# unanan/UNet_Nested4Tiny_Objects_Keypoints

Measured on AMD Instinct MI355X. Metric: images/sec (train step) UNet++ L=4 256x256, higher is better.
Workload: dtype f32

## Files before the change

### include/unetpp_hip.h

```cpp
#ifndef UNETPP_HIP_H
#define UNETPP_HIP_H

#include <stdint.h>

#ifdef __cplusplus
extern "C" {
#endif

#define UNETPP_ABI_VERSION 12
#define UNETPP_MAX_VIEWS 8

#define UNETPP_OK 0
#define UNETPP_EINVAL (-1)
#define UNETPP_ELAUNCH (-2)

typedef struct unetpp_view {
  float* ptr;
  int32_t C, c_off, c_len;
  int32_t Hs, Ws;
  int32_t sy, sx, oy, ox;
  const float* scale;
  const float* shift;
  const float* gate;
  int32_t relu;
// ... 292 lines not shown
                      const int32_t* chunk_segment, int64_t n_chunks, int64_t count, double decay, float* count_dev,
                      const double* hyper_dev, int32_t* done, void* stream);

#define UNETPP_WARP_PARAMS 16
#define UNETPP_WARP_MAX_C 8
#define UNETPP_STORE_U8 0
#define UNETPP_STORE_F32 1

int unetpp_warp_batch(const void* store, int32_t store_type, int64_t M, int32_t Hs, int32_t Ws, int32_t C,
                      const int64_t* index, int32_t N, const float* params, const float* mul, const float* add,
                      float fill, float* out, int32_t Ho, int32_t Wo, const float* labels, int32_t S,
                      float* labels_out, uint8_t* inside, void* stream);

typedef struct unetpp_augment {
  float p_flip_h, p_flip_v;
  int32_t rot90;
  float max_deg;
  float scale_lo, scale_hi;
  float max_tx, max_ty;
  float gain_lo, gain_hi;
  float max_bias;
  int32_t reserved;
} unetpp_augment;

int unetpp_augment_draw(float* params, int32_t N, uint64_t seed, int32_t Hs, int32_t Ws, int32_t Ho, int32_t Wo,
                        const unetpp_augment* augment, void* stream);

#define UNETPP_SCENE_MAX_VARIANTS 8
#define UNETPP_SCENE_FLIP_X 1
#define UNETPP_SCENE_FLIP_Y 2
#define UNETPP_SCENE_TRANSPOSE 4

typedef struct unetpp_scene_rect {
  int32_t frame;
  int32_t oy, ox;
  int32_t y_lo, y_hi, x_lo, x_hi;
  int32_t reserved;
} unetpp_scene_rect;

int unetpp_scene_stitch(const float* tiles, int32_t n_tiles, int32_t K, int32_t C, int32_t Th, int32_t Tw,
                        const int32_t* variants, const unetpp_scene_rect* rects, const unetpp_scene_rect* rects_dev,
                        float* out, int32_t S, int32_t H, int32_t W, void* stream);


int64_t unetpp_peaks_workspace_bytes(int32_t M, int32_t H, int32_t W);
int unetpp_peaks_detect(const float* maps, int32_t M, int32_t H, int32_t W, float threshold, int32_t radius,
                        int32_t refine, int32_t cap, float* xy, float* score, int32_t* count, void* workspace,
                        void* stream);

int unetpp_detect_match(const float* xy, const int32_t* n_pred, const int32_t* order, int32_t S, int32_t C, int32_t cap,
                        const float* labels, const int32_t* label_class, int32_t L, float tolerance, int32_t* pred_label,
                        int32_t* label_pred, int32_t* stats, void* stream);

#ifdef __cplusplus
}
#endif
#endif
```

### unet_nested4tiny_objects_keypoints_amd/_lib.py

```python
from __future__ import annotations

import ctypes as C
import os
import subprocess

_PKG_DIR = os.path.dirname(os.path.abspath(__file__))
_REPO = os.path.dirname(_PKG_DIR)
LIB_PATH = os.environ.get("UNETPP_LIB", os.path.join(_PKG_DIR, "libunetpp_hip.so"))
CSRC = os.path.join(_PKG_DIR, "csrc")
INCLUDE = os.path.join(_REPO, "include")
SOURCES = ("gemm_pix.hip", "gemm_fast.hip", "gemm_pw.hip", "gemm_pw_bf16.hip", "gemm_wino.hip", "gemm_bf16.hip", "gemm_bf16_dma.hip", "wgrad_bf16.hip", "pointwise_bf16.hip", "keypoints.hip", "weight_image.hip", "wgrad.hip", "wgrad_fast.hip", "wgrad_dma.hip", "wgrad_pw.hip", "wgrad_wino.hip", "first_layer.hip", "pointwise.hip", "caller.hip", "optim.hip", "validate.hip", "average.hip", "loader.hip", "scene.hip",
           "detect.hip")
HEADERS = ("common.h", "gemm_units.h", "wgrad_reduce.h", "lds_asm.h", "bf16_common.h", "dropout.h", "bn_fused.h",
           "wino_experiments.h", "dma_experiments.h", "heads_mean.h")
MAX_VIEWS = 8
ABI_VERSION = 12
EXTRA_FLAGS = {"gemm_wino.hip": ("-fno-slp-vectorize",), "wgrad_wino.hip": ("-fno-slp-vectorize",)}
GEMM_DIRECT = 1
GEMM_BF16 = 2


class View(C.Structure):
    _fields_ = [
        ("ptr", C.c_void_p),
        ("C", C.c_int32), ("c_off", C.c_int32), ("c_len", C.c_int32),
        ("Hs", C.c_int32), ("Ws", C.c_int32),
        ("sy", C.c_int32), ("sx", C.c_int32), ("oy", C.c_int32), ("ox", C.c_int32),
        ("scale", C.c_void_p), ("shift", C.c_void_p), ("gate", C.c_void_p),
        ("relu", C.c_int32), ("accumulate", C.c_int32), ("gate_sum", C.c_int32), ("reserved", C.c_int32),
    ]


class BnFused(C.Structure):
    _fields_ = [
        ("gamma", C.c_void_p), ("beta", C.c_void_p), ("running_mean", C.c_void_p), ("running_var", C.c_void_p),
        ("mean", C.c_void_p), ("invstd", C.c_void_p), ("scale", C.c_void_p), ("shift", C.c_void_p),
        ("count", C.c_int64), ("eps", C.c_float), ("momentum", C.c_float),
    ]


class GemmDesc(C.Structure):
    _fields_ = [
        ("N", C.c_int32), ("H", C.c_int32), ("W", C.c_int32),
        ("taps", C.c_int32), ("n_in", C.c_int32), ("n_out", C.c_int32),
        ("flags", C.c_int32), ("reserved", C.c_int32),
        ("inp", View * MAX_VIEWS), ("out", View * MAX_VIEWS),
        ("weight", C.c_void_p), ("bias", C.c_void_p), ("stats_partial", C.c_void_p),
        ("weight_image", C.c_void_p),
        ("bn", BnFused),
    ]


class WeightSrc(C.Structure):
    _fields_ = [
        ("src", C.c_void_p),
        ("s_t", C.c_int64), ("s_k", C.c_int64), ("s_ko", C.c_int64), ("s_n", C.c_int64), ("s_no", C.c_int64),
        ("k_inner", C.c_int32), ("n_inner", C.c_int32), ("flip", C.c_int32), ("reserved", C.c_int32),
    ]


class PackJob(C.Structure):
    _fields_ = [
        ("src", WeightSrc),
        ("image", C.c_void_p),
        ("taps", C.c_int32), ("flags", C.c_int32), ("n_in", C.c_int32), ("n_out", C.c_int32),
# ... 125 lines not shown
    "unetpp_bn_bwd_reduce_pool": (C.c_int, [_P, _P, _P, _P, _P, _P, _P, _P, _I32, _I32, _I32, _I32, _P, _P]),
    "unetpp_bn_bwd_apply_pool": (C.c_int, [_P, _P, _P, _P, _P, _P, _P, _P, _P, _P, _P, _I32, _I32, _I32, _I32, _P, _P]),
    "unetpp_head_fwd": (C.c_int, [_P, _P, _P, _I32, _I32, _I32, _I32, _I32, _F, _U64, _P, _P, _P, _P]),
    "unetpp_head_bwd_blocks": (_I64, [_I64]),
    "unetpp_head_bwd": (C.c_int, [_P, _P, _P, _P, _I32, _I32, _I32, _I32, _I32, _F, _U64, _P, _P, _P, _I32, _I32, _P, _P]),
    "unetpp_sum_partials": (C.c_int, [_P, _I64, _I64, _P, _P]),
    "unetpp_focal_bce_blocks": (_I64, [_I64]),
    "unetpp_focal_bce": (C.c_int, [_P, _P, _I64, _I64, _F, _P, _P, _P, _P]),
    "unetpp_focal_bce_heads": (C.c_int, [C.POINTER(FocalHeads), _P, _I64, _I64, _F, _P, _P, _P]),
    "unetpp_heads_mean_fwd": (C.c_int, [C.POINTER(HeadsMean), _I32, _I32, _I32, _I32, _I32, _P, _P]),
    "unetpp_heads_mean_fwd_bf16": (C.c_int, [C.POINTER(HeadsMean), _I32, _I32, _I32, _I32, _I32, _P, _P]),
    "unetpp_bn_eval_coeffs_stats": (C.c_int, [_P, _P, _P, _P, _F, _I32, _P, _P, _P, _P, _P]),
    "unetpp_bn_frozen_bwd_blocks": (_I64, [_I64, _I32]),
    "unetpp_bn_frozen_bwd": (C.c_int, [_P, _P, _P, _P, _P, _P, _P, _P, _I32, _I32, _I32, _I32, _P, _P, _P]),
    "unetpp_bn_frozen_bwd_blocks_bf16": (_I64, [_I64, _I32]),
    "unetpp_bn_frozen_bwd_bf16": (C.c_int, [_P, _P, _P, _P, _P, _P, _P, _P, _I32, _I32, _I32, _I32, _P, _P, _P]),
    "unetpp_copy_jobs": (C.c_int, [_P, _I32, _I64, _P]),
    "unetpp_heatmap_workspace_bytes": (_I64, [_I32, _I32, _I32]),
    "unetpp_create_heatmap": (C.c_int, [_P, _I32, _I32, _I32, _I32, _F, _P, _P, _P]),
    "unetpp_bilinear2x_fwd": (C.c_int, [_P, _I32, _I32, _I32, _I32, _P, _P]),
    "unetpp_bilinear2x_bwd": (C.c_int, [_P, _I32, _I32, _I32, _I32, _P, _I32, _P]),
    "unetpp_nchw_to_nhwc": (C.c_int, [_P, _I32, _I32, _I32, _I32, _P, _P]),
    "unetpp_nhwc_to_nchw": (C.c_int, [_P, _I32, _I32, _I32, _I32, _P, _P]),
    "unetpp_affine_relu_pool_bf16": (C.c_int, [_P, _P, _P, _I32, _I32, _I32, _I32, _I32, _P, _P, _P, _P]),
    "unetpp_bn_bwd_blocks_bf16": (_I64, [_I64, _I32]),
    "unetpp_bn_bwd_reduce_bf16": (C.c_int, [_P, _P, _P, _P, _P, _P, _P, _P, _I32, _I32, _I32, _I32, _P, _P]),
    "unetpp_bn_bwd_apply_bf16": (C.c_int, [_P, _P, _P, _P, _P, _P, _P, _P, _P, _P, _P, _I32, _I32, _I32, _I32, _P, _P]),
    "unetpp_head_fwd_bf16": (C.c_int, [_P, _P, _P, _I32, _I32, _I32, _I32, _I32, _F, _U64, _P, _P, _P, _P]),
    "unetpp_first_layer_dgrad_bf16": (C.c_int, [_P, _P, _I32, _I32, _I32, _I32, _I32, _P, _P]),
    "unetpp_maxpool_bwd_bf16": (C.c_int, [_P, _P, _I32, _I32, _I32, _I32, _P, _P, _P]),
    "unetpp_bilinear2x_fwd_bf16": (C.c_int, [_P, _I32, _I32, _I32, _I32, _P, _P]),
    "unetpp_bilinear2x_bwd_bf16": (C.c_int, [_P, _I32, _I32, _I32, _I32, _P, _I32, _P, _P]),
    "unetpp_heatmap_pattern_workspace_bytes": (_I64, [_I32, _I32, _I32, _I32]),
    "unetpp_heatmap_pattern": (C.c_int, [_P, _I32, _I32, _P, _P, _I32, _I32, _I32, _F, _P, _P, _P]),
    "unetpp_keypoints_workspace_bytes": (_I64, [_I32, _I32, _I32, _I32]),
    "unetpp_keypoints_extract": (C.c_int, [_I32, _P, _I32, _I32, _I32, _P, _I32, _I32, _I32, _P, _P, _P, _P, _P]),
    "unetpp_head_bwd_bf16": (C.c_int, [_P, _P, _P, _P, _I32, _I32, _I32, _I32, _I32, _F, _U64, _P, _P, _P, _I32, _I32, _P, _P]),
    "unetpp_optim_chunk_elems": (_I64, []),
    "unetpp_optim_step": (C.c_int, [_I32, _I32, _P, _I32, _P, _I64, _P, _P, _P, _P]),
    "unetpp_optim_upload": (C.c_int, [_P, _P, _I64, _P]),
    "unetpp_match_points": (C.c_int, [_P, _P, _I32, _I32, _I32, _I32, _P, _I32, _P, _P, _P, _P, _P, _P, _P]),
    "unetpp_avg_update": (C.c_int, [_I32, _I32, _P, _I32, _P, _I64, _I64, C.c_double, _P, _P, _P, _P]),
    "unetpp_grad_norm": (C.c_int, [_P, _I32, _P, _I64, _P, _P]),
    "unetpp_optim_step_clip": (C.c_int, [_I32, _I32, _P, _I32, _P, _I64, _P, _P, _P, _P, _P, _P]),
    "unetpp_grad_scale": (C.c_int, [_P, _I32, _P, _I64, _P, _F, _P, _P]),
    "unetpp_warp_batch": (C.c_int, [_P, _I32, _I64, _I32, _I32, _I32, _P, _I32, _P, _P, _P, _F, _P, _I32, _I32, _P, _I32,
                                    _P, _P, _P]),
    "unetpp_augment_draw": (C.c_int, [_P, _I32, _U64, _I32, _I32, _I32, _I32, C.POINTER(AugmentDesc), _P]),
    "unetpp_scene_stitch": (C.c_int, [_P, _I32, _I32, _I32, _I32, _I32, C.POINTER(C.c_int32), C.POINTER(SceneRect), _P, _P,
                                      _I32, _I32, _I32, _P]),
    "unetpp_peaks_workspace_bytes": (_I64, [_I32, _I32, _I32]),
    "unetpp_peaks_detect": (C.c_int, [_P, _I32, _I32, _I32, _F, _I32, _I32, _I32, _P, _P, _P, _P, _P]),
    "unetpp_detect_match": (C.c_int, [_P, _P, _P, _I32, _I32, _I32, _P, _P, _I32, _F, _P, _P, _P, _P]),
}

_LIB = None


def source_hash() -> str:
    import hashlib
    h = hashlib.sha256()
    for path in [os.path.join(CSRC, s) for s in SOURCES + HEADERS] + [os.path.join(INCLUDE, "unetpp_hip.h")]:
        with open(path, "rb") as f:
            h.update(f.read())
    return h.hexdigest()[:16]


def build_library(force: bool = False, verbose: bool = False, out_path: str = None, obj_dir: str = None) -> str:
    srcs = [os.path.join(CSRC, s) for s in SOURCES]
    deps = srcs + [os.path.join(CSRC, h) for h in HEADERS] + [os.path.join(INCLUDE, "unetpp_hip.h")]
    lib_path = out_path or LIB_PATH
    if not force and os.path.exists(lib_path) and all(os.path.getmtime(lib_path) >= os.path.getmtime(d) for d in deps):
        return lib_path
    hipcc = os.environ.get("HIPCC", "/opt/rocm/bin/hipcc")
    common = [hipcc, "--offload-arch=gfx950", "-O3", "-std=c++17", "-fPIC", "-I", INCLUDE, "-I", CSRC]
    obj_dir = obj_dir or os.path.join(_REPO, "build", "obj")
    os.makedirs(obj_dir, exist_ok=True)
    jobs = []
    for src in SOURCES:
        obj = os.path.join(obj_dir, src.replace(".hip", ".o"))
        cmd = common + list(EXTRA_FLAGS.get(src, ())) + ["-c", os.path.join(CSRC, src), "-o", obj]
        if verbose:
            print(" ".join(cmd))
        jobs.append((obj, cmd, subprocess.Popen(cmd)))
    for obj, cmd, proc in jobs:
        if proc.wait() != 0:
            raise subprocess.CalledProcessError(proc.returncode, cmd)
    staged = os.path.join(obj_dir, os.path.basename(lib_path) + ".link")
    link = [hipcc, "--offload-arch=gfx950", "-shared", "-fPIC", "-o", staged] + [j[0] for j in jobs]
    if verbose:
        print(" ".join(link))
    subprocess.run(link, check=True)
    os.replace(staged, lib_path)
    if out_path is None:
        global _LIB
        _LIB = None
    return lib_path


def lib():
    global _LIB
    if _LIB is None:
        if not os.path.exists(LIB_PATH):
            raise RuntimeError(
                "unetpp HIP library not built: %s is missing. Run `python -c 'import __graft_entry__ as g; g.build()'` "
                "(there is no CPU fallback for this path)." % LIB_PATH)
# ... 37 lines not shown
```

### unet_nested4tiny_objects_keypoints_amd/engine.py

```python
from __future__ import annotations

import os

from typing import Dict, List, Optional, Tuple

import torch

from . import ops
from .ops import V


USE_PACK_PLAN = os.environ.get("UNETPP_NO_PACK_PLAN") is None
USE_GROUPED_DGRAD = os.environ.get("UNETPP_NO_GROUPED_DGRAD") is None
USE_PLAN_COPIES = os.environ.get("UNETPP_NO_PLAN_COPIES") is None
_A1_MATERIALIZE_BYTES = int(float(os.environ.get("UNETPP_BF16_A1_MAX_MB", "80")) * (1 << 20))
_A1_MATERIALIZE_BYTES_F32 = int(float(os.environ.get("UNETPP_F32_A1_MAX_MB", "80")) * (1 << 20))


def _empty(n, like):
    return torch.empty(n, dtype=torch.float32, device=like.device)


def _packed(w, t, k, n, dstr, sstr, flip=False):
    dst = _empty(t * k * n, w)
    ops.pack_weight(dst, w, t, k, n, dstr, sstr, flip=flip)
    return dst


def pack_conv_fwd(w):
    co, ci, kh, kw = w.shape
    t = kh * kw
    return ops.WSrc(w, t, ci, co, s_t=1, s_k=t, s_n=ci * t,
                    pack=lambda: _packed(w, t, ci, co, (ci * co, co, 1), (1, t, ci * t)))


def pack_conv_dgrad(w):
    co, ci, kh, kw = w.shape
    t = kh * kw
    return ops.WSrc(w, t, co, ci, s_t=1, s_k=ci * t, s_n=t, flip=True,
                    pack=lambda: _packed(w, t, co, ci, (co * ci, ci, 1), (1, ci * t, t), flip=True))


def pack_conv_dgrad_slice(w, c_off, c_len):
    co, ci, kh, kw = w.shape
    t = kh * kw
    flat = w.reshape(-1)[c_off * t:]
    return ops.WSrc(flat, t, co, c_len, s_t=1, s_k=ci * t, s_n=t, flip=True,
                    pack=lambda: _packed(w[:, c_off:c_off + c_len].contiguous(), t, co, c_len, (co * c_len, c_len, 1),
                                         (1, c_len * t, t), flip=True))


def pack_deconv_fwd(w):
    ci, co = w.shape[0], w.shape[1]
    return ops.WSrc(w, 1, ci, 4 * co, s_t=0, s_k=4 * co, s_n=4, s_no=1, n_inner=co,
                    pack=lambda: _packed(w, 4, ci, co, (co, 4 * co, 1), (1, 4 * co, 4)))


def pack_deconv_dgrad(w):
    ci, co = w.shape[0], w.shape[1]
    return ops.WSrc(w, 1, 4 * co, ci, s_t=0, s_k=4, s_ko=1, k_inner=co, s_n=4 * co,
                    pack=lambda: _packed(w, 4, co, ci, (co * ci, ci, 1), (1, 4, 4 * co)))


def tile_bias4(b):
    co = b.numel()
    plan = ops.current_plan()
    if plan is not None and USE_PLAN_COPIES and b.is_contiguous():
        dst, ready = plan.copy_for(("bias4", b.data_ptr()) + ops.phase_tag(plan.phase), plan.phase, (b.data_ptr(), co),
                                   lambda: (_empty(4 * co, b), [b], [(b, 0, 0, 4, co, 0, co)]))
# ... 355 lines not shown
                               _new_grad(bn.weight), _new_grad(bn.bias), pool=pool_grad)
    if not (bn.weight.requires_grad or bn.bias.requires_grad):
        return ops.bn_frozen_backward(d_act, y, scale, shift, None, None, d_act, pool=pool_grad, want_sums=False)
    return ops.bn_frozen_backward(d_act, y, scale, shift, mean, invstd, d_act, _new_grad(bn.weight), _new_grad(bn.bias),
                                  pool=pool_grad)


def _pair_bwd(blk, r: _PairRec, d_out, in_targets: Optional[List[V]], b, grads, pre_gated=False, pool_grad=None,
              flush=None, in_slice: Optional[Tuple[int, int]] = None):
    conv1, conv2 = getattr(blk.conv1, "0"), getattr(blk.conv2, "0")
    h, w = r.h, r.w
    if blk.is_batchnorm:
        bn1, bn2 = getattr(blk.conv1, "1"), getattr(blk.conv2, "1")
        grads[bn2.weight], grads[bn2.bias] = _bn_bwd(bn2, r.bn2, r.frozen2, d_out, r.y2, pool_grad)
        dy2 = V(d_out)
        mean, invstd, scale, shift = r.bn1
        if r.a1 is not None:
            _conv_wgrad(conv2, [V(r.a1)], [dy2], b, h, w, grads)
        else:
            _conv_wgrad(conv2, [V(r.y1, scale=scale, shift=shift, relu=True)], [dy2], b, h, w, grads)
        if flush is not None:
            flush()
        d_a1 = torch.empty_like(r.y1)
        ops.gemm_fwd(b, h, w, 9, [dy2], [V(d_a1)], pack_conv_dgrad(conv2.weight.detach()))
        grads[bn1.weight], grads[bn1.bias] = _bn_bwd(bn1, r.bn1, r.frozen1, d_a1, r.y1, None)
        dy1 = V(d_a1)
    else:
        dy2 = V(d_out) if pre_gated else V(d_out, gate=r.out)
        _conv_wgrad(conv2, [V(r.a1)], [dy2], b, h, w, grads)
        if flush is not None:
            flush()
        d_a1 = torch.empty_like(r.a1)
        ops.gemm_fwd(b, h, w, 9, [dy2], [V(d_a1, gate=r.a1)], pack_conv_dgrad(conv2.weight.detach()))
        dy1 = V(d_a1)
    _conv_wgrad(conv1, r.ins, [dy1], b, h, w, grads)
    if flush is not None:
        flush()
    if in_targets is not None:
        if dy1.t.dtype == torch.bfloat16 and in_targets[0].t.dtype == torch.float32:
            ops.first_layer_dgrad_bf16(dy1.t, conv1.weight.detach(), in_targets[0].t)
        elif in_slice is not None:
            ops.gemm_fwd(b, h, w, 9, [dy1], in_targets, pack_conv_dgrad_slice(conv1.weight.detach(), in_slice[0], in_slice[1]))
        else:
            ops.gemm_fwd(b, h, w, 9, [dy1], in_targets, pack_conv_dgrad(conv1.weight.detach()))
    return dy1


def _up_bwd(upmod, is_deconv, u: _UpRec, d_up, d_src, accumulate, gate, b, grads):
    hs, ws = u.h, u.w
    if is_deconv:
        ci, co = upmod.weight.shape[0], upmod.weight.shape[1]
        dw = _new_grad(upmod.weight)
        db = _new_grad(upmod.bias)
        ops.wgrad(b, hs, ws, 1, [V(u.src)], _phase_views(d_up), dw, (0, 4 * co, 4, 1), db, n_inner=co)
        grads[upmod.weight], grads[upmod.bias] = dw, db
        ops.gemm_fwd(b, hs, ws, 1, _phase_views(d_up), [V(d_src, accumulate=accumulate, gate=gate, gate_sum=True)],
                     pack_deconv_dgrad(upmod.weight.detach()))
    else:
        conv = getattr(upmod, "1")
        _conv_wgrad(conv, [V(u.interp)], [V(d_up)], b, 2 * hs, 2 * ws, grads)
        d_interp = torch.empty_like(u.interp)
        ops.gemm_fwd(b, 2 * hs, 2 * ws, 1, [V(d_up)], [V(d_interp)], pack_conv_dgrad(conv.weight.detach()))
        ops.bilinear2x_bwd(d_interp, d_src, accumulate, gate)


def _grouped_weights(model, refresh=False, plan=None):
    cache = getattr(model, "_grouped_dgrad_w", None)
    d = model.depth
    if cache is None or refresh:
        fresh = {}
        for i in range(d - 1):
            for jj in range(d - 1 - i):
                ws = [getattr(getattr(model, "up_concat%d%d" % (i, jc)).conv.conv1, "0").weight.detach()
                      for jc in range(jj + 1, d - i)]
                f = ws[0].shape[0]
                parts = [w[:, (1 + jj) * f:(2 + jj) * f] for w in ws]
                old = None if cache is None else cache.get((i, jj))
                if old is not None and not (old.device == parts[0].device and old.dtype == parts[0].dtype):
                    old = None
                if plan is not None and all(w.is_contiguous() and w.dtype == torch.float32 for w in ws):
                    key, sig = ("grouped", i, jj), tuple(w.data_ptr() for w in ws)
                    if old is not None and plan.knows_copy(key, "bwd", sig + (old.data_ptr(),)):
                        plan.copy_for(key, "bwd", sig + (old.data_ptr(),), None)
                        fresh[(i, jj)] = old
                        continue
                    buf = old if old is not None else torch.empty((len(ws) * f, f) + tuple(ws[0].shape[2:]),
                                                                   dtype=ws[0].dtype, device=ws[0].device)
                    t = ws[0].shape[2] * ws[0].shape[3]
                    items = [(w, (1 + jj) * f * t, q * f * f * t, f, f * t, w.shape[1] * t, f * t) for q, w in enumerate(ws)]
                    plan.copy_for(key, "bwd", sig + (buf.data_ptr(),), lambda: (buf, list(ws), items))
                    old = buf
                if old is not None:
                    torch.cat(parts, 0, out=old)
                    fresh[(i, jj)] = old
                else:
                    fresh[(i, jj)] = torch.cat(parts, 0).contiguous()
        cache = fresh
        model._grouped_dgrad_w = cache
    return cache


def backward_impl(model, s: _Saved, d_outs, want_input_grad: bool, grad_sink=None):
    if USE_GROUPED_DGRAD:
        _grouped_weights(model, refresh=True, plan=_plan_of(model) if (USE_PACK_PLAN and USE_PLAN_COPIES) else None)
    if not USE_PACK_PLAN:
        return _backward_impl(model, s, d_outs, want_input_grad, grad_sink)
# ... 140 lines not shown
```

### unet_nested4tiny_objects_keypoints_amd/ops.py

```python
from __future__ import annotations

import ctypes as C
import functools
import os
from dataclasses import dataclass
from typing import Optional, Sequence

import torch

from . import _lib
from ._lib import MAX_VIEWS, GemmDesc, PackJob, View, WeightSrc, WgradDesc, check


def _stream():
    return C.c_void_p(torch.cuda.current_stream().cuda_stream)


class LaunchTimer:

    def __init__(self):
        self.launches = []
        self.regions = []
        self.want_launches = True
        self.want_regions = True
# ... 404 lines not shown
                check(lib.unetpp_gemm_pack_weight_image(C.byref(d), _ptr(image), _stream()),
                      "unetpp_gemm_pack_weight_image")
            d.weight_image = image.data_ptr()
    if d.weight_image is None and from_src:
        packed = weight.packed()
        d.weight = packed.data_ptr()
    acc = sum(v.c_len for v in d.out[:d.n_out] if v.accumulate) + sum(v.c_len for v in d.out[:d.n_out] if v.gate)
    _timed_call(None, 2.0 * n * h * w * taps * k * nc,
                lambda: check(_lib.lib().unetpp_gemm_fwd(C.byref(d), _stream()), "unetpp_gemm_fwd"),
                (2.0 if d.flags & _lib.GEMM_BF16 else 4.0) * n * h * w * (k + nc + acc))


def first_layer_dgrad_bf16(dy: torch.Tensor, weight: torch.Tensor, dx: torch.Tensor) -> None:
    n, h, w, co = dy.shape
    ci = dx.shape[3]
    _need(dy, "dy", torch.bfloat16)
    _need(weight, "weight")
    _need(dx, "dx")
    if tuple(weight.shape) != (co, ci, 3, 3) or tuple(dx.shape[:3]) != (n, h, w):
        raise ValueError("shape mismatch")
    check(_lib.lib().unetpp_first_layer_dgrad_bf16(_ptr(dy), _ptr(weight), n, h, w, ci, co, _ptr(dx), _stream()),
          "unetpp_first_layer_dgrad_bf16")


def pack_weight(dst: torch.Tensor, src: torch.Tensor, t: int, k: int, n: int, dstr, sstr, flip: bool = False) -> None:
    _need(dst, "pack dst")
    _need(src, "pack src")
    check(_lib.lib().unetpp_pack_weight(_ptr(dst), _ptr(src), t, k, n, dstr[0], dstr[1], dstr[2],
                                        sstr[0], sstr[1], sstr[2], int(flip), _stream()), "unetpp_pack_weight")


def wgrad(n: int, h: int, w: int, taps: int, xs: Sequence[V], dys: Sequence[V], dw: Optional[torch.Tensor],
          dw_strides, db: Optional[torch.Tensor], n_inner: Optional[int] = None, target_blocks: int = 256,
          direct: bool = False) -> _lib.WgradSizes:
    lib = _lib.lib()
    d = WgradDesc()
    d.N, d.H, d.W, d.taps = n, h, w, taps
    d.n_x, d.n_dy = len(xs), len(dys)
    k = sum(v.fill(d.x[i]) for i, v in enumerate(xs))
    nc = sum(v.fill(d.dy[i]) for i, v in enumerate(dys))
    d.flags = (_lib.GEMM_DIRECT if (direct or not USE_WINOGRAD) else 0) | _storage_flag(dys, xs)
    plan = _lib.WgradSizes()
    check(lib.unetpp_wgrad_plan(C.byref(d), target_blocks, C.byref(plan)), "unetpp_wgrad_plan")
    slabs = torch.empty(plan.slab_floats, dtype=torch.float32, device=xs[0].t.device)
    d.n_split, d.slabs = plan.n_split, slabs.data_ptr()
    _timed_call(None, 2.0 * n * h * w * taps * k * nc,
                lambda: check(lib.unetpp_wgrad(C.byref(d), _stream()), "unetpp_wgrad"),
                (2.0 if d.flags & _lib.GEMM_BF16 else 4.0) * n * h * w * (k + nc))
    if n_inner is None:
        n_inner = nc
    check(lib.unetpp_wgrad_finish(_ptr(slabs), plan.n_split, plan.planes, k, nc, n_inner, _ptr(dw), dw_strides[0],
                                  dw_strides[1], dw_strides[2], dw_strides[3], _ptr(db), _stream()), "unetpp_wgrad_finish")
    return plan


def bn_finalize(partial, n_blocks, c, count, gamma, beta, eps, momentum, running_mean, running_var):
    dev = partial.device
    mean, invstd, scale, shift = (torch.empty(c, dtype=torch.float32, device=dev) for _ in range(4))
    check(_lib.lib().unetpp_bn_finalize(_ptr(partial), n_blocks, c, count, _ptr(gamma), _ptr(beta), eps, momentum,
                                        _ptr(running_mean), _ptr(running_var), _ptr(mean), _ptr(invstd), _ptr(scale),
                                        _ptr(shift), _stream()), "unetpp_bn_finalize")
    return mean, invstd, scale, shift


def bn_eval_coeffs(gamma, beta, running_mean, running_var, eps):
    c = gamma.numel()
    scale, shift = (torch.empty(c, dtype=torch.float32, device=gamma.device) for _ in range(2))
    check(_lib.lib().unetpp_bn_eval_coeffs(_ptr(gamma), _ptr(beta), _ptr(running_mean), _ptr(running_var), eps, c,
                                           _ptr(scale), _ptr(shift), _stream()), "unetpp_bn_eval_coeffs")
    return scale, shift


def bn_eval_coeffs_stats(gamma, beta, running_mean, running_var, eps):
    c = gamma.numel()
    mean, invstd, scale, shift = (torch.empty(c, dtype=torch.float32, device=gamma.device) for _ in range(4))
    check(_lib.lib().unetpp_bn_eval_coeffs_stats(_ptr(gamma), _ptr(beta), _ptr(running_mean), _ptr(running_var), eps, c,
                                                 _ptr(scale), _ptr(shift), _ptr(mean), _ptr(invstd), _stream()),
          "unetpp_bn_eval_coeffs_stats")
    return mean, invstd, scale, shift


def _is_bf16(t):
    return t.dtype == torch.bfloat16


def affine_relu_pool(y, scale, shift, relu, act, pooled, pool_idx):
    n, h, w, c = y.shape
    if _is_bf16(y):
        check(_lib.lib().unetpp_affine_relu_pool_bf16(_ptr(y), _ptr(scale), _ptr(shift), int(relu), n, h, w, c, _ptr(act),
                                                      _ptr(pooled), _ptr(pool_idx), _stream()),
              "unetpp_affine_relu_pool_bf16")
        return
    check(_lib.lib().unetpp_affine_relu_pool(_ptr(y), _ptr(scale), _ptr(shift), int(relu), n, h, w, c, _ptr(act),
                                             _ptr(pooled), _ptr(pool_idx), _stream()), "unetpp_affine_relu_pool")


def maxpool_bwd(d_pooled, pool_idx, d_act, gate=None):
    n, h, w, c = d_act.shape
    if _is_bf16(d_act):
        check(_lib.lib().unetpp_maxpool_bwd_bf16(_ptr(d_pooled), _ptr(pool_idx), n, h, w, c, _ptr(d_act), _ptr(gate), _stream()),
              "unetpp_maxpool_bwd_bf16")
        return
    if gate is not None:
        raise ValueError("the fused ReLU mask is a bf16-storage option")
    check(_lib.lib().unetpp_maxpool_bwd(_ptr(d_pooled), _ptr(pool_idx), n, h, w, c, _ptr(d_act), _stream()),
          "unetpp_maxpool_bwd")
# ... 548 lines not shown
```

Measured before the change: 1716.

## Fuse transposed-conv weight gradient and data gradient into one pointwise backward kernel

Adds a HIP kernel that computes the 2x2 stride-2 deconvolution's weight/bias gradient and its input gradient in a single pass. Each tile of the upsampled gradient and the source activation is read once and feeds both the wgrad MFMA accumulation and the dgrad MFMA with its gate/accumulate epilogue. Previously these were two launches that each read the same activations. In exchange it uses a large LDS footprint, an eight-wave in-block reduction and per-shape template variants. It applies only to f32 levels whose width is a multiple of 16 and whose weights fit in LDS.

```diff
diff --git a/include/unetpp_hip.h b/include/unetpp_hip.h
--- a/include/unetpp_hip.h
+++ b/include/unetpp_hip.h
@@ -368,6 +368,10 @@
                         const float* labels, const int32_t* label_class, int32_t L, float tolerance, int32_t* pred_label,
                         int32_t* label_pred, int32_t* stats, void* stream);
 
+
+int unetpp_pw_bwd_fused(const unetpp_wgrad_desc* d, const float* weight, const unetpp_view* d_src, int32_t launch,
+                        void* stream);
+
 #ifdef __cplusplus
 }
 #endif
diff --git a/unet_nested4tiny_objects_keypoints_amd/_lib.py b/unet_nested4tiny_objects_keypoints_amd/_lib.py
--- a/unet_nested4tiny_objects_keypoints_amd/_lib.py
+++ b/unet_nested4tiny_objects_keypoints_amd/_lib.py
@@ -10,7 +10,7 @@
 CSRC = os.path.join(_PKG_DIR, "csrc")
 INCLUDE = os.path.join(_REPO, "include")
 SOURCES = ("gemm_pix.hip", "gemm_fast.hip", "gemm_pw.hip", "gemm_pw_bf16.hip", "gemm_wino.hip", "gemm_bf16.hip", "gemm_bf16_dma.hip", "wgrad_bf16.hip", "pointwise_bf16.hip", "keypoints.hip", "weight_image.hip", "wgrad.hip", "wgrad_fast.hip", "wgrad_dma.hip", "wgrad_pw.hip", "wgrad_wino.hip", "first_layer.hip", "pointwise.hip", "caller.hip", "optim.hip", "validate.hip", "average.hip", "loader.hip", "scene.hip",
-           "detect.hip")
+           "detect.hip", "pw_bwd_fused.hip")
 HEADERS = ("common.h", "gemm_units.h", "wgrad_reduce.h", "lds_asm.h", "bf16_common.h", "dropout.h", "bn_fused.h",
            "wino_experiments.h", "dma_experiments.h", "heads_mean.h")
 MAX_VIEWS = 8
@@ -242,6 +242,7 @@
     "unetpp_peaks_workspace_bytes": (_I64, [_I32, _I32, _I32]),
     "unetpp_peaks_detect": (C.c_int, [_P, _I32, _I32, _I32, _F, _I32, _I32, _I32, _P, _P, _P, _P, _P]),
     "unetpp_detect_match": (C.c_int, [_P, _P, _P, _I32, _I32, _I32, _P, _P, _I32, _F, _P, _P, _P, _P]),
+    "unetpp_pw_bwd_fused": (C.c_int, [C.POINTER(WgradDesc), _P, C.POINTER(View), _I32, _P]),
 }
 
 _LIB = None
diff --git a/unet_nested4tiny_objects_keypoints_amd/csrc/pw_bwd_fused.hip b/unet_nested4tiny_objects_keypoints_amd/csrc/pw_bwd_fused.hip
--- /dev/null
+++ b/unet_nested4tiny_objects_keypoints_amd/csrc/pw_bwd_fused.hip
@@ -0,0 +1,362 @@
+#include "common.h"
+#include "lds_asm.h"
+
+namespace unetpp {
+namespace {
+
+constexpr int kFusedThreads = 512;
+constexpr size_t kFusedLdsBytes = 4 * 34 * 256 * sizeof(float);
+
+struct FusedArgs {
+  unetpp_wgrad_desc d;
+  unetpp_view out;
+  const float* weight;
+  int ci, co;
+  int kb_count, nb_count;
+  int nt_store;
+  long rows;
+};
+
+__device__ __forceinline__ long view_origin(const unetpp_view& v) {
+  return (static_cast<long>(v.oy) * v.Ws + v.ox) * v.C + v.c_off;
+}
+
+typedef unsigned u32x4v __attribute__((vector_size(16)));
+constexpr unsigned kBeyondRow = 0x80000000u;
+__device__ __forceinline__ __amdgpu_buffer_rsrc_t row_rsrc(const float* row, int row_bytes) {
+  return __builtin_amdgcn_make_buffer_rsrc(const_cast<float*>(row), 0, row_bytes, 0x00020000);
+}
+__device__ __forceinline__ f32x4 row_load4(__amdgpu_buffer_rsrc_t rs, unsigned lane_off, unsigned tile_off) {
+  return __builtin_bit_cast(f32x4, __builtin_amdgcn_raw_buffer_load_b128(rs, static_cast<int>(lane_off), static_cast<int>(tile_off), 0));
+}
+
+template <int NCB, bool FULL, bool GATE, bool ACC>
+__global__ __launch_bounds__(kFusedThreads, 2) void pw_bwd_fused_kernel(const FusedArgs a) {
+  constexpr int CO = 128 / NCB, NCH = 4 / NCB;
+  extern __shared__ __attribute__((aligned(16))) float fused_lds[];
+  const unetpp_wgrad_desc& d = a.d;
+  const int tid = threadIdx.x, lane = tid & 63, t16 = lane & 15, g = lane >> 4;
+  const int wave = __builtin_amdgcn_readfirstlane(tid >> 6);
+  constexpr int n_ps = 8;
+  const int ps = wave;
+  const int blocks = a.kb_count * a.nb_count, n_wg = gridDim.x;
+  int wg = blockIdx.x;
+  if ((n_wg & 7) == 0) wg = (blockIdx.x & 7) * (n_wg >> 3) + (blockIdx.x >> 3);
+  const int split = wg / blocks, sb = wg - split * blocks;
+  const int kb = sb / a.nb_count, nb = sb - kb * a.nb_count;
+  const int cb0 = sb * NCB;
+
+  for (int i = tid; i < 8 * NCH * NCB * 64; i += kFusedThreads) {
+    const int l = i & 63, blk = i >> 6;
+    const int cb = blk % NCB, qg = blk / NCB;
+    const int k = 16 * qg + 4 * (l >> 4), ph = k / CO, c = k - ph * CO;
+    const int n = 16 * (cb0 + cb) + (l & 15);
+    const float* wp = a.weight + (static_cast<long>(n) * CO + c) * 4 + ph;
+    *reinterpret_cast<f32x4*>(fused_lds + i * 4) = f32x4{wp[0], wp[4], wp[8], wp[12]};
+  }
+  __syncthreads();
+
+  const int W = d.W, H = d.H;
+  const unetpp_view& X0 = d.x[0];
+  const unetpp_view& Y0 = d.dy[0];
+  const unetpp_view& O = a.out;
+  const long x_row = static_cast<long>(X0.sy) * X0.Ws * X0.C, y_row = static_cast<long>(Y0.sy) * Y0.Ws * Y0.C;
+  const int x_px = X0.sx * X0.C, y_px = Y0.sx * Y0.C;
+  const int x_row_bytes = static_cast<int>(x_row) * 4, y_row_bytes = static_cast<int>(y_row) * 4;
+  const long x_org = view_origin(X0);
+  const int xa_c = static_cast<int>(x_org) + 64 * kb + 4 * t16;
+  int yb_c[2];
+#pragma unroll
+  for (int h = 0; h < 2; ++h) {
+    const int col = 128 * nb + 64 * h + 4 * t16, ph = col / CO;
+    yb_c[h] = static_cast<int>(view_origin(d.dy[ph])) + (col - ph * CO);
+  }
+  int yph[4];
+#pragma unroll
+  for (int p = 0; p < 4; ++p) yph[p] = static_cast<int>(view_origin(d.dy[p]));
+  const int o_px = O.sx * O.C;
+  const unsigned a_lane = static_cast<unsigned>(g * x_px + xa_c) * 4u;
+  const unsigned b_lane[2] = {static_cast<unsigned>(g * y_px + yb_c[0]) * 4u, static_cast<unsigned>(g * y_px + yb_c[1]) * 4u};
+  const bool o_gsum = O.gate_sum != 0;
+
+  const long parts = static_cast<long>(d.n_split) * n_ps, part = static_cast<long>(split) * n_ps + ps;
+  const long r0 = a.rows * part / parts, r1 = a.rows * (part + 1) / parts;
+
+  f32x4 acc[4][2][4];
+#pragma unroll
+  for (int m = 0; m < 4; ++m)
+#pragma unroll
+    for (int h = 0; h < 2; ++h)
+#pragma unroll
+      for (int q = 0; q < 4; ++q) acc[m][h][q] = f32x4{0.f, 0.f, 0.f, 0.f};
+  f32x4 dbs[2] = {f32x4{0.f, 0.f, 0.f, 0.f}, f32x4{0.f, 0.f, 0.f, 0.f}};
+
+  f32x4 X[8];
+  auto load_x = [&](auto chunk_c, long r, int x0) {
+    constexpr int chunk = decltype(chunk_c)::v;
+    const __amdgpu_buffer_rsrc_t yr = row_rsrc(Y0.ptr + r * y_row, y_row_bytes);
+    const unsigned lo = (FULL || x0 + t16 < W) ? static_cast<unsigned>(t16 * y_px + 4 * g) * 4u : kBeyondRow;
+#pragma unroll
+    for (int q = 0; q < 8; ++q) {
+      const int k0 = 128 * chunk + 16 * q, ph = k0 / CO, c = k0 - ph * CO;
+      X[q] = row_load4(yr, lo, static_cast<unsigned>(x0 * y_px + yph[ph] + c) * 4u);
+    }
+  };
+
+  const unsigned wa = lds_offset(fused_lds) + lane * 16;
+  long r = r0;
+  int x0 = 0;
+  if (r < r1) load_x(IC<0>{}, r, x0);
+  while (r < r1) {
+    const int n = static_cast<int>(r / H), y = static_cast<int>(r - static_cast<long>(n) * H);
+    const int x_this = x0;
+    const bool pv = FULL || x0 + t16 < W;
+    const __amdgpu_buffer_rsrc_t xr = row_rsrc(X0.ptr + r * x_row, x_row_bytes), yr = row_rsrc(Y0.ptr + r * y_row, y_row_bytes);
+    f32x4 A[4], B[4][2];
+#pragma unroll
+    for (int s = 0; s < 4; ++s) {
+      const unsigned lo = (FULL || x0 + 4 * s + g < W) ? a_lane : kBeyondRow;
+      A[s] = row_load4(xr, lo, static_cast<unsigned>((x0 + 4 * s) * x_px) * 4u);
+    }
+
+    const long o_tile = view_pixel_offset(O, n, y, x0) + 16 * cb0;
+    const __amdgpu_buffer_rsrc_t orr = row_rsrc(O.ptr + o_tile, 64 * o_px);
+    const __amdgpu_buffer_rsrc_t grr = row_rsrc(GATE ? O.gate + o_tile : O.ptr, 64 * o_px);
+    const unsigned oo = pv ? static_cast<unsigned>(t16 * o_px + 4 * g) * 4u : kBeyondRow;
+    constexpr bool kEarlyOld = NCB < 4;
+    f32x4 old[NCB];
+#pragma unroll
+    for (int cb = 0; cb < NCB; ++cb) {
+      if constexpr (ACC && kEarlyOld) old[cb] = row_load4(orr, oo, 64 * cb);
+    }
+
+    f32x4 dacc[NCB];
+#pragma unroll
+    for (int cb = 0; cb < NCB; ++cb) dacc[cb] = f32x4{0.f, 0.f, 0.f, 0.f};
+    static_for<NCH>([&](auto cc) {
+      constexpr int chunk = decltype(cc)::v;
+      if constexpr (chunk > 0) load_x(cc, r, x0);
+      const unsigned wb = wa + static_cast<unsigned>(chunk * (8 * NCB * 1024));
+      f32x4 wf[2];
+      asm volatile("ds_read_b128 %0, %1" : "=v"(wf[0]) : "v"(wb) : "memory");
+      static_for<8 * NCB>([&](auto ic) {
+        constexpr int i = decltype(ic)::v, q = i / NCB, cb = i % NCB;
+        if constexpr (i + 1 < 8 * NCB) {
+          asm volatile("ds_read_b128 %0, %1 offset:%2" : "=v"(wf[(i + 1) & 1]) : "v"(wb), "n"((i + 1) * 1024) : "memory");
+          asm volatile("s_waitcnt lgkmcnt(1)" : "+v"(wf[i & 1]));
+        } else {
+          asm volatile("s_waitcnt lgkmcnt(0)" : "+v"(wf[i & 1]));
+        }
+#pragma unroll
+        for (int e = 0; e < 4; ++e) dacc[cb] = __builtin_amdgcn_mfma_f32_16x16x4f32(wf[i & 1][e], X[q][e], dacc[cb], 0, 0, 0);
+      });
+    });
+
+    f32x4 gt[NCB];
+#pragma unroll
+    for (int cb = 0; cb < NCB; ++cb) {
+      if constexpr (GATE) gt[cb] = row_load4(grr, oo, 64 * cb);
+      if constexpr (ACC && !kEarlyOld) old[cb] = row_load4(orr, oo, 64 * cb);
+    }
+#pragma unroll
+    for (int cb = 0; cb < NCB; ++cb) {
+      f32x4 v = dacc[cb];
+      if constexpr (GATE) {
+#pragma unroll
+        for (int e = 0; e < 4; ++e) v[e] = (o_gsum || gt[cb][e] > 0.f) ? v[e] : 0.f;
+      }
+      if constexpr (ACC) {
+#pragma unroll
+        for (int e = 0; e < 4; ++e) v[e] += old[cb][e];
+      }
+      if constexpr (GATE) {
+#pragma unroll
+        for (int e = 0; e < 4; ++e) v[e] = (!o_gsum || gt[cb][e] > 0.f) ? v[e] : 0.f;
+      }
+      dacc[cb] = v;
+    }
+
+    auto load_b = [&]() {
+#pragma unroll
+      for (int s = 0; s < 4; ++s) {
+        const bool in_row = FULL || x_this + 4 * s + g < W;
+        const unsigned l0 = in_row ? b_lane[0] : kBeyondRow, l1 = in_row ? b_lane[1] : kBeyondRow;
+        B[s][0] = row_load4(yr, l0, static_cast<unsigned>((x_this + 4 * s) * y_px) * 4u);
+        B[s][1] = row_load4(yr, l1, static_cast<unsigned>((x_this + 4 * s) * y_px) * 4u);
+      }
+    };
+    if constexpr (kEarlyOld) load_b();
+#pragma unroll
+    for (int cb = 0; cb < NCB; ++cb) {
+      if (a.nt_store) __builtin_amdgcn_raw_buffer_store_b128(__builtin_bit_cast(u32x4v, dacc[cb]), orr, static_cast<int>(oo), 64 * cb, 2);
+      else __builtin_amdgcn_raw_buffer_store_b128(__builtin_bit_cast(u32x4v, dacc[cb]), orr, static_cast<int>(oo), 64 * cb, 0);
+    }
+    if constexpr (!kEarlyOld) load_b();
+
+    x0 += 16;
+    if (x0 >= W) {
+      x0 = 0;
+      ++r;
+    }
+    if (r < r1) load_x(IC<0>{}, r, x0);
+
+#pragma unroll
+    for (int s = 0; s < 4; ++s) {
+      if (FULL || x_this + 4 * s < W) {
+        const f32x4 av = A[s], b0 = B[s][0], b1 = B[s][1];
+#pragma unroll
+        for (int e = 0; e < 4; ++e) {
+          dbs[0][e] += b0[e];
+          dbs[1][e] += b1[e];
+        }
+#pragma unroll
+        for (int m = 0; m < 4; ++m)
+#pragma unroll
+          for (int q = 0; q < 4; ++q) {
+            acc[m][0][q] = __builtin_amdgcn_mfma_f32_16x16x4f32(av[m], b0[q], acc[m][0][q], 0, 0, 0);
+            acc[m][1][q] = __builtin_amdgcn_mfma_f32_16x16x4f32(av[m], b1[q], acc[m][1][q], 0, 0, 0);
+          }
+      }
+    }
+  }
+
+  float* red_lds = fused_lds;
+  for (int half = n_ps >> 1; half >= 1; half >>= 1) {
+    __syncthreads();
+    if (ps >= half && ps < 2 * half) {
+      float* rg = red_lds + (ps - half) * (34 * 256) + lane * 4;
+#pragma unroll
+      for (int m = 0; m < 4; ++m)
+#pragma unroll
+        for (int h = 0; h < 2; ++h)
+#pragma unroll
+          for (int q = 0; q < 4; ++q) *reinterpret_cast<f32x4*>(rg + ((m * 2 + h) * 4 + q) * 256) = acc[m][h][q];
+      *reinterpret_cast<f32x4*>(rg + 32 * 256) = dbs[0];
+      *reinterpret_cast<f32x4*>(rg + 33 * 256) = dbs[1];
+    }
+    __syncthreads();
+    if (ps < half) {
+      const float* rg = red_lds + ps * (34 * 256) + lane * 4;
+#pragma unroll
+      for (int m = 0; m < 4; ++m)
+#pragma unroll
+        for (int h = 0; h < 2; ++h)
+#pragma unroll
+          for (int q = 0; q < 4; ++q) acc[m][h][q] += *reinterpret_cast<const f32x4*>(rg + ((m * 2 + h) * 4 + q) * 256);
+      dbs[0] += *reinterpret_cast<const f32x4*>(rg + 32 * 256);
+      dbs[1] += *reinterpret_cast<const f32x4*>(rg + 33 * 256);
+    }
+  }
+  if (ps != 0) return;
+
+  const int Kw = a.ci, Nw = 4 * a.co;
+  float* slab = d.slabs + static_cast<long>(split) * (static_cast<long>(Kw) + 1) * Nw;
+#pragma unroll
+  for (int m = 0; m < 4; ++m)
+#pragma unroll
+    for (int h = 0; h < 2; ++h)
+#pragma unroll
+      for (int rr = 0; rr < 4; ++rr) {
+        const int k = 64 * kb + 4 * (4 * g + rr) + m, nn = 128 * nb + 64 * h + 4 * t16;
+        *reinterpret_cast<f32x4*>(slab + static_cast<long>(k) * Nw + nn) =
+            f32x4{acc[m][h][0][rr], acc[m][h][1][rr], acc[m][h][2][rr], acc[m][h][3][rr]};
+      }
+  if (kb == 0) {
+#pragma unroll
+    for (int h = 0; h < 2; ++h) {
+      f32x4 v = dbs[h];
+#pragma unroll
+      for (int e = 0; e < 4; ++e) {
+        v[e] += __shfl_xor(v[e], 16);
+        v[e] += __shfl_xor(v[e], 32);
+      }
+      if (g == 0) *reinterpret_cast<f32x4*>(slab + static_cast<long>(Kw) * Nw + 128 * nb + 64 * h + 4 * t16) = v;
+    }
+  }
+}
+
+bool fused_plain(const unetpp_view& v) {
+  return v.scale == nullptr && v.shift == nullptr && v.gate == nullptr && !v.relu && ((v.C | v.c_off | v.c_len) & 3) == 0 &&
+         (reinterpret_cast<uintptr_t>(v.ptr) & 15) == 0;
+}
+
+bool fused_shape(const unetpp_wgrad_desc* d, const float* weight, const unetpp_view* out, FusedArgs& a) {
+  if (d == nullptr || weight == nullptr || out == nullptr) return false;
+  if (d->N <= 0 || d->H <= 0 || d->W <= 0 || d->taps != 1 || (d->flags & UNETPP_GEMM_BF16) != 0) return false;
+  if (d->n_x != 1 || d->n_dy != 4 || d->slabs == nullptr || d->n_split < 1 || d->n_split > 4096) return false;
+  if ((reinterpret_cast<uintptr_t>(weight) & 3) != 0 || (reinterpret_cast<uintptr_t>(d->slabs) & 15) != 0) return false;
+  const unetpp_view& x = d->x[0];
+  if (!view_ok(x) || !view_covers(x, d->H, d->W) || !fused_plain(x) || x.Hs != x.sy * d->H) return false;
+  a.ci = x.c_len;
+  a.co = d->dy[0].c_len;
+  if ((a.ci & 63) != 0 || (a.co != 32 && a.co != 64 && a.co != 128)) return false;
+  for (int i = 0; i < 4; ++i) {
+    const unetpp_view& y = d->dy[i];
+    if (!view_ok(y) || !view_covers(y, d->H, d->W) || !fused_plain(y) || y.c_len != a.co || y.Hs != y.sy * d->H) return false;
+    if (y.ptr != d->dy[0].ptr || y.C != d->dy[0].C || y.Hs != d->dy[0].Hs || y.Ws != d->dy[0].Ws || y.sy != d->dy[0].sy ||
+        y.sx != d->dy[0].sx)
+      return false;
+  }
+  const unetpp_view& y0 = d->dy[0];
+  if (static_cast<long>(x.sy) * x.Ws * x.C * 4 >= 0x7fffffffL || static_cast<long>(y0.sy) * y0.Ws * y0.C * 4 >= 0x7fffffffL ||
+      static_cast<long>(out->sx) * out->C * 64 >= 0x7fffffffL)
+    return false;
+  if (!view_ok(*out) || !view_covers(*out, d->H, d->W) || out->c_len != a.ci || out->scale != nullptr || out->relu != 0) return false;
+  if (((out->C | out->c_off) & 3) != 0 || (reinterpret_cast<uintptr_t>(out->ptr) & 15) != 0 ||
+      (reinterpret_cast<uintptr_t>(out->gate) & 15) != 0)
+    return false;
+  a.kb_count = a.ci >> 6;
+  a.nb_count = a.co >> 5;
+  if (static_cast<long>(a.kb_count) * a.nb_count * d->n_split > 0x7fffffffL) return false;
+  a.rows = static_cast<long>(d->N) * d->H;
+  return true;
+}
+
+template <int NCB, bool FULL, bool GATE, bool ACC>
+int launch_fused(const FusedArgs& a, dim3 grid, hipStream_t st) {
+  static bool raised[64] = {};
+  int dev = 0;
+  if (hipGetDevice(&dev) != hipSuccess || dev < 0 || dev >= 64) return UNETPP_ELAUNCH;
+  if (!raised[dev]) {
+    if (hipFuncSetAttribute(reinterpret_cast<const void*>(&pw_bwd_fused_kernel<NCB, FULL, GATE, ACC>), hipFuncAttributeMaxDynamicSharedMemorySize,
+                            static_cast<int>(kFusedLdsBytes)) != hipSuccess)
+      return UNETPP_ELAUNCH;
+    raised[dev] = true;
+  }
+  hipLaunchKernelGGL((pw_bwd_fused_kernel<NCB, FULL, GATE, ACC>), grid, dim3(kFusedThreads), kFusedLdsBytes, st, a);
+  return launch_status();
+}
+
+}
+}
+
+using namespace unetpp;
+
+extern "C" int unetpp_pw_bwd_fused(const unetpp_wgrad_desc* d, const float* weight, const unetpp_view* d_src, int32_t launch,
+                                   void* stream) {
+  FusedArgs a;
+  if (!fused_shape(d, weight, d_src, a)) return UNETPP_EINVAL;
+  if (launch == 0) return UNETPP_OK;
+  a.d = *d;
+  a.out = *d_src;
+  a.weight = weight;
+  const long out_bytes = static_cast<long>(d->N) * d->H * d->W * a.ci * 4;
+  a.nt_store = static_cast<int>(opt_value(OPT_PW_NT, out_bytes >= (64L << 20) ? 1 : 0));
+  const dim3 grid(static_cast<unsigned>(d->n_split) * static_cast<unsigned>(a.kb_count * a.nb_count));
+  hipStream_t st = static_cast<hipStream_t>(stream);
+  note_kernel("pw_bwd_fused_kernel");
+  const bool full = (d->W & 15) == 0;
+  const bool gate = d_src->gate != nullptr, accum = d_src->accumulate != 0;
+#define UNETPP_FUSED_EPI(NCB, FULL) \
+  return gate ? (accum ? launch_fused<NCB, FULL, true, true>(a, grid, st) : launch_fused<NCB, FULL, true, false>(a, grid, st)) \
+              : (accum ? launch_fused<NCB, FULL, false, true>(a, grid, st) : launch_fused<NCB, FULL, false, false>(a, grid, st));
+#define UNETPP_FUSED_CASE(NCB) \
+  if (full) { UNETPP_FUSED_EPI(NCB, true) } else { UNETPP_FUSED_EPI(NCB, false) }
+  switch (a.co) {
+    case 32: UNETPP_FUSED_CASE(4)
+    case 64: UNETPP_FUSED_CASE(2)
+    default: UNETPP_FUSED_CASE(1)
+  }
+#undef UNETPP_FUSED_CASE
+#undef UNETPP_FUSED_EPI
+}
diff --git a/unet_nested4tiny_objects_keypoints_amd/engine.py b/unet_nested4tiny_objects_keypoints_amd/engine.py
--- a/unet_nested4tiny_objects_keypoints_amd/engine.py
+++ b/unet_nested4tiny_objects_keypoints_amd/engine.py
@@ -15,6 +15,11 @@
 USE_PLAN_COPIES = os.environ.get("UNETPP_NO_PLAN_COPIES") is None
 _A1_MATERIALIZE_BYTES = int(float(os.environ.get("UNETPP_BF16_A1_MAX_MB", "80")) * (1 << 20))
 _A1_MATERIALIZE_BYTES_F32 = int(float(os.environ.get("UNETPP_F32_A1_MAX_MB", "80")) * (1 << 20))
+USE_PW_FUSED_BWD = os.environ.get("UNETPP_PW_FUSED_BWD", "1") != "0"
+
+
+def _pw_fused_level(ci, co, ws):
+    return ws % 16 == 0 and (4 * co * ci + ci) * 4 <= 148 * 1024
 
 
 def _empty(n, like):
@@ -476,6 +481,11 @@
         ci, co = upmod.weight.shape[0], upmod.weight.shape[1]
         dw = _new_grad(upmod.weight)
         db = _new_grad(upmod.bias)
+        if (USE_PW_FUSED_BWD and _pw_fused_level(ci, co, ws) and d_up.dtype == torch.float32 and
+                ops.pw_bwd_fused(b, hs, ws, V(u.src), d_up, upmod.weight.detach(),
+                                 V(d_src, accumulate=accumulate, gate=gate, gate_sum=True), dw, db)):
+            grads[upmod.weight], grads[upmod.bias] = dw, db
+            return
         ops.wgrad(b, hs, ws, 1, [V(u.src)], _phase_views(d_up), dw, (0, 4 * co, 4, 1), db, n_inner=co)
         grads[upmod.weight], grads[upmod.bias] = dw, db
         ops.gemm_fwd(b, hs, ws, 1, _phase_views(d_up), [V(d_src, accumulate=accumulate, gate=gate, gate_sum=True)],
diff --git a/unet_nested4tiny_objects_keypoints_amd/ops.py b/unet_nested4tiny_objects_keypoints_amd/ops.py
--- a/unet_nested4tiny_objects_keypoints_amd/ops.py
+++ b/unet_nested4tiny_objects_keypoints_amd/ops.py
@@ -480,6 +480,47 @@
     check(lib.unetpp_wgrad_finish(_ptr(slabs), plan.n_split, plan.planes, k, nc, n_inner, _ptr(dw), dw_strides[0],
                                   dw_strides[1], dw_strides[2], dw_strides[3], _ptr(db), _stream()), "unetpp_wgrad_finish")
     return plan
+
+
+def pw_bwd_fused(n: int, h: int, w: int, src: V, d_up: torch.Tensor, weight: torch.Tensor, d_src: V,
+                 dw: torch.Tensor, db: torch.Tensor, target_blocks: int = 256) -> bool:
+    lib = _lib.lib()
+    ci, co = weight.shape[0], weight.shape[1]
+    _need(weight, "weight")
+    if tuple(weight.shape) != (ci, co, 2, 2) or d_up.dim() != 4 or tuple(d_up.shape) != (n, 2 * h, 2 * w, d_up.shape[3]):
+        raise ValueError("shape mismatch")
+    dys = [V(d_up, c_len=co, sy=2, sx=2, oy=a, ox=b) for a in (0, 1) for b in (0, 1)]
+    d = WgradDesc()
+    d.N, d.H, d.W, d.taps = n, h, w, 1
+    d.n_x, d.n_dy = 1, 4
+    k = src.fill(d.x[0])
+    nc = sum(v.fill(d.dy[i]) for i, v in enumerate(dys))
+    if src.t.dtype != torch.float32 or d_up.dtype != torch.float32 or d_src.t.dtype != torch.float32:
+        return False
+    d.flags = 0
+    out = View()
+    if d_src.fill(out) != ci or k != ci:
+        raise ValueError("src / d_src must have the weight's %d input channels" % ci)
+    plan = _lib.WgradSizes()
+    if lib.unetpp_wgrad_plan(C.byref(d), target_blocks, C.byref(plan)) == 0 and plan.kernel == b"wgrad_pw_kernel":
+        n_split = plan.n_split
+    else:
+        n_split = max(1, min(target_blocks // max(1, (ci // 64) * (co // 32)), n * h, 4096))
+    slabs = torch.empty(n_split * (ci + 1) * nc, dtype=torch.float32, device=d_up.device)
+    d.n_split, d.slabs = n_split, slabs.data_ptr()
+    if lib.unetpp_pw_bwd_fused(C.byref(d), _ptr(weight), C.byref(out), 0, None) != 0:
+        return False
+    _need(dw, "dw")
+    _need(db, "db")
+    if tuple(dw.shape) != (ci, co, 2, 2) or db.numel() != co:
+        raise ValueError("gradient shape mismatch")
+    acc = (ci if d_src.accumulate else 0) + (ci if d_src.gate is not None else 0)
+    _timed_call("pw_bwd_fused_kernel", 4.0 * n * h * w * ci * nc,
+                lambda: check(lib.unetpp_pw_bwd_fused(C.byref(d), _ptr(weight), C.byref(out), 1, _stream()),
+                              "unetpp_pw_bwd_fused"), 4.0 * n * h * w * (2 * ci + nc + acc))
+    check(lib.unetpp_wgrad_finish(_ptr(slabs), n_split, 1, ci, nc, co, _ptr(dw), 0, 4 * co, 4, 1, _ptr(db), _stream()),
+          "unetpp_wgrad_finish")
+    return True
 
 
 def bn_finalize(partial, n_blocks, c, count, gamma, beta, eps, momentum, running_mean, running_var):
```

After: 1725 (median of 6 runs). About the same (+0.5%).
